# jetuk/pycllp

Hardware: AMD Instinct MI355X
Metric: LPs solved/sec (higher is better)
Workload: dtype f64

## Files before the change

pycllp_amd/csrc/ipm_group.inc:

```

#ifndef PYCLLP_SPLITJ
#define PYCLLP_SPLITJ 6
#endif
#ifndef PYCLLP_GRAM_UNROLL
#define PYCLLP_GRAM_UNROLL 4
#endif
#ifndef PYCLLP_AT_RB
#define PYCLLP_AT_RB 4
#endif
#ifndef PYCLLP_A_CB
#define PYCLLP_A_CB 8
#endif
#ifndef PYCLLP_SOLVE_PRIO
#define PYCLLP_SOLVE_PRIO 2
#endif
#ifndef PYCLLP_FACTOR_PRIO
#define PYCLLP_FACTOR_PRIO 2
#endif
#ifndef PYCLLP_FACTOR_PRIO_HSD
#define PYCLLP_FACTOR_PRIO_HSD 3
#endif
#ifndef PYCLLP_WPB
#define PYCLLP_WPB 8
#endif
// ... 51 lines not shown
    static constexpr int GTAB_OFF = AIMG + ND;
    __device__ static void fill_gram_table(double* lds, int tid, int nthreads) {
        if constexpr (MP == 32) {
            unsigned short* tab = (unsigned short*)(lds + GTAB_OFF);
            for (int i = tid; i < GROWS * 64; i += nthreads)
                tab[i] = (unsigned short)(i < GRAM_INSTS * 64 ? gram_store(i >> 6, i & 63) : gram_wrap(i & 63));
        }
    }
    static constexpr int SHARED = GTAB_OFF + GTAB;
    static constexpr int WSZ = G * SLAB + STAGE_SZ;
    static constexpr size_t lds_bytes(int wpb) { return sizeof(double) * (size_t)(SHARED + wpb * WSZ); }
    __host__ __device__ static constexpr int kpos(int j) { return (j & 3) * KS + (j >> 2); }
};

template <int MP>
__device__ __forceinline__ double grp_sum(double v) {
    asm volatile("" : "+v"(v));
    v += dpp_d<0xB1>(v);
    v += dpp_d<0x4E>(v);
    v += dpp_d<0x141>(v);
    v += dpp_d<0x140>(v);
    if (MP == 32) v = row_pair_sum(v);
    return v;
}
template <int MP>
__device__ __forceinline__ double grp_max(double v) {
    v = fmax(v, dpp_d<0xB1>(v));
    v = fmax(v, dpp_d<0x4E>(v));
    v = fmax(v, dpp_d<0x141>(v));
    v = fmax(v, dpp_d<0x140>(v));
    if (MP == 32) v = row_pair_max(v);
    return v;
}
template <int MP>
__device__ __forceinline__ double grp_bcast(double v, int k, int grp) {
    if (MP == 32) {
        const double a = readlane_d(v, k), b = readlane_d(v, 32 + k);
        return grp ? b : a;
    } else {
        const double a = readlane_d(v, k), b = readlane_d(v, 16 + k), c = readlane_d(v, 32 + k), d = readlane_d(v, 48 + k);
        return (grp & 2) ? ((grp & 1) ? d : c) : ((grp & 1) ? b : a);
    }
}

template <int MP, int NP, bool SL = false>
struct GWave {
    using G_ = GeoG<MP, NP, SL>;
    static constexpr int G = G_::G, NCG = G_::NCG, NCD = G_::NCD, ND = G_::ND, JB = G_::JB, KS = G_::KS, AS = G_::AS, MS = G_::MS;

    const double* Aimg;
    static constexpr bool COLB = MP == 32 && NP <= 96;
    static constexpr bool ROWB = COLB && SL;
    static constexpr bool CARRY = COLB || MP == 16;
    unsigned rb[ROWB ? 16 : 1];
    unsigned xb[COLB ? 16 : 1];
    double* slab;
    double* slab0;
    double* stage;
    int lane, gl, grp, m, n;

    __device__ __forceinline__ int ogl() const { int g = gl; asm volatile("" : "+v"(g)); return g; }

    __device__ __forceinline__ void load_own_row(double (&out)[MP]) const {
        typedef double double2_t __attribute__((ext_vector_type(2)));
        if constexpr (ROWB) {
#pragma unroll
            for (int p2 = 0; p2 < MP / 2; p2++) {
                const double2_t t = *(const __attribute__((address_space(3))) double2_t*)(size_t)rb[p2];
                out[2 * p2] = t[0]; out[2 * p2 + 1] = t[1];
            }
            return;
        }
        const int g = ogl();
        const double2_t* rp = (const double2_t*)(slab + g * MS);
        const int g15 = G_::SWZ ? (g & 15) : 0;
#pragma unroll
        for (int p2 = 0; p2 < MP / 2; p2++) {
            const double2_t t = rp[p2 ^ g15];
            out[2 * p2] = t[0]; out[2 * p2 + 1] = t[1];
        }
    }

    template <bool STAGED = false>
    __device__ __forceinline__ void At_times(double u, double (&out)[NCG]) const {
        const int g = ogl();
        double ur[2] = {u, u};
        const __attribute__((address_space(3))) double* ub = nullptr;
        if constexpr (STAGED) {
            stage[grp * MP + g] = u;
            wave_lds_sync();
            unsigned uba = lds_addr(stage + grp * MP);
            asm volatile("" : "+v"(uba));
            ub = (const __attribute__((address_space(3))) double*)(size_t)uba;
        } else if constexpr (MP == 32) {
            ur[0] = top_row_d(u); ur[1] = bottom_row_d(u);
        }
        const double* ac = Aimg + g;
        constexpr int RB = PYCLLP_AT_RB, NB = MP / RB;
        double a0[RB][NCD], a1[RB][NCD], u0[RB], u1[RB];
#define AT_LOAD(A_, U_, I0)                                                                     \
    static_for<0, RB>([&](auto ic_) {                                                           \
        constexpr int ii = decltype(ic_)::value, i_ = (I0) + ii;                                \
        if constexpr (STAGED) U_[ii] = ub[i_ + tok];                                            \
        else U_[ii] = row_bcast<(i_ & 15)>(ur[i_ >> 4]);                                        \
        _Pragma("unroll") for (int q = 0; q < NCD; q++) A_[ii][q] = ac[i_ * AS + MP * q + tok]; \
    });
#define AT_USE(A_, U_)                                                                          \
    _Pragma("unroll") for (int ii = 0; ii < RB; ii++) {                                         \
        asm volatile("" : "+v"(U_[ii]));                                                        \
        _Pragma("unroll") for (int q = 0; q < NCD; q++) asm volatile("" : "+v"(A_[ii][q]));     \
    }                                                                                           \
    asm volatile("" : "+v"(tok));                                                               \
    _Pragma("unroll") for (int ii = 0; ii < RB; ii++)                                           \
        _Pragma("unroll") for (int q = 0; q < NCD; q++) out[q] = fma(A_[ii][q], U_[ii], out[q]); \
    _Pragma("unroll") for (int q = 0; q < NCD; q++) asm volatile("" : "+v"(out[q]));
#pragma unroll
        for (int q = 0; q < NCG; q++) out[q] = 0.0;
        if (SL) out[NCG - 1] = u;
        int tok = 0;
        asm volatile("" : "+v"(tok));
        AT_LOAD(a0, u0, 0)
        static_for<0, NB / 2>([&](auto bc) {
            constexpr int b2 = 2 * decltype(bc)::value;
            AT_LOAD(a1, u1, (b2 + 1) * RB)
            AT_USE(a0, u0)
            if constexpr (b2 + 2 < NB) { AT_LOAD(a0, u0, (b2 + 2) * RB) }
            AT_USE(a1, u1)
        });
#undef AT_LOAD
#undef AT_USE
        if constexpr (STAGED) wave_lds_sync();
    }
// ... 79 lines not shown
                    acc[0] = __builtin_amdgcn_mfma_f64_4x4x4f64(ad[0], a[0], acc[0], 0, 0, 0);
                    acc[1] = __builtin_amdgcn_mfma_f64_4x4x4f64(ad[1], a[1], acc[1], 0, 0, 0);
                    acc[2] = __builtin_amdgcn_mfma_f64_4x4x4f64(ad[0], p3, acc[2], 0, 0, 0);
                    acc[3] = __builtin_amdgcn_mfma_f64_4x4x4f64(ad[1], p7, acc[3], 0, 0, 0);
                    acc[4] = __builtin_amdgcn_mfma_f64_4x4x4f64(top ? ad[0] : ad[1], p2, acc[4], 0, 0, 0);
                }
            }
            int lo_ = lane;
            asm volatile("" : "+v"(lo_));
            if constexpr (LATE) {
                const unsigned short* tab2 = (const unsigned short*)(Aimg + G_::GTAB_OFF) + lo_;
#pragma unroll
                for (int r = 0; r < GRAM_INSTS; r++) so[r] = tab2[64 * r];
            }
            const unsigned sga = lds_addr(sg);
#pragma unroll
            for (int r = 0; r < GRAM_INSTS; r++) *(__attribute__((address_space(3))) double*)(size_t)(sga + so[r]) = acc[r];
            const int kg2 = lo_ >> 4, c0 = (lo_ & 15) ^ (kg2 << 1);
            double* e0 = sg + kg2 * G_::MS + c0;
            double* e1 = sg + kg2 * G_::MS + (c0 ^ 8);
#pragma unroll
            for (int r4 = 0; r4 < 4; r4++) ((r4 & 1) ? e1 : e0)[(16 + 4 * r4) * G_::MS + 16 * (r4 >> 1)] = acc10[r4];
        } else {
            double4_t acc = (double4_t){0.0, 0.0, 0.0, 0.0};
#pragma unroll PYCLLP_GRAM_UNROLL
            for (int s0 = 0; s0 < KS; s0 += SC) {
#pragma unroll
                for (int ss = 0; ss < SC; ss++) {
                    const int s = s0 + ss;
                    const double xk = AX ? px[s] : 0.0, dk = pd[s], tk = pt[s];
                    const double a = arow[4 * s];
                    if (AX) axp[0] = fma(a, xk, axp[0]);
                    adp[0] = fma(a, tk, adp[0]);
                    acc = __builtin_amdgcn_mfma_f64_16x16x4f64(a * dk, a, acc, 0, 0, 0);
                }
            }
            int lo_ = lane;
            asm volatile("" : "+v"(lo_));
            const int kg2 = lo_ >> 4, cc2 = lo_ & 15;
#pragma unroll
            for (int r4 = 0; r4 < 4; r4++) sg[G_::sidx(kg2 + 4 * r4, cc2)] = acc[r4];
        }
        if constexpr (MP == 32) {
            if (AX) ax = quad_sum2(axp[0], axp[1]);
            ad = quad_sum2(adp[0], adp[1]);
        } else {
            if (AX) ax = quad_sum(axp[0]);
            ad = quad_sum(adp[0]);
        }
    }

    __device__ __forceinline__ static double top_row_of(double u) { return top_row_d(u); }

    template <bool RELF = false>
    __device__ __forceinline__ bool factor_dpp(double (&W)[MP], double beta2, double floor_, bool live, double& rdiag,
                                               const double* fl = nullptr) const {
        return factor_sweep<RELF, 0>(W, beta2, floor_, live, rdiag, fl, nullptr);
    }
    template <bool RELF = false, int NR>
    __device__ __forceinline__ bool factor_dpp_fwd(double (&W)[MP], double beta2, double floor_, bool live, double& rdiag,
                                                   double (&r)[NR], const double* fl = nullptr) const {
        return factor_sweep<RELF, NR>(W, beta2, floor_, live, rdiag, fl, r);
    }
    template <int OP, int NR>
    __device__ __forceinline__ static void fwd_bottom_op(const double (&W)[MP], double* r, const double* so, double* a) {
        if constexpr (OP >= 0 && OP < 16) {
#pragma unroll
            for (int i = 0; i < NR; i++) dot_step<OP, 0xA>(a[i], so[i], W[OP]);
        } else if constexpr (OP == 16) {
#pragma unroll
            for (int i = 0; i < NR; i++) r[i] -= a[i];
        } else if constexpr (OP > 16 && OP < 32) {
#pragma unroll
            for (int i = 0; i < NR; i++) fwd_step<OP - 17, 0xA>(r[i], W[OP - 1]);
        }
    }
    template <bool RELF, int NR>
    __device__ __forceinline__ bool factor_sweep(double (&W)[MP], double beta2, double floor_, bool live, double& rdiag,
                                                 const double* fl, double* r) const {
        rdiag = 1.0;
        constexpr int PRIO_ = RELF ? PYCLLP_FACTOR_PRIO_HSD : PYCLLP_FACTOR_PRIO;
        if constexpr (PRIO_ != 0) __builtin_amdgcn_s_setprio(PRIO_);
        const int go = ogl();
        (void)go;
        constexpr int NR1 = NR ? NR : 1;
        double so[NR1], acc[NR1];
#pragma unroll
        for (int i = 0; i < NR1; i++) { so[i] = 0.0; acc[i] = 0.0; }
        double ymax = 0.0;
        static_for<0, MP>([&](auto jc) {
            constexpr int j = decltype(jc)::value;
            const double u = W[j];
            double src = u;
            if constexpr (MP == 32 && j < 16) src = top_row_of(u);
            const double piv = bcast64<j % 16>(src);
            if constexpr (NR > 0 && MP == 32 && j > 16) fwd_bottom_op<2 * (j - 16) - 1, NR>(W, r, so, acc);
            const double aD = RELF ? max_abs<false>(piv, fl[j]) : max_abs<true>(piv, floor_);
            double rD = fast_rcp(aD);
            if constexpr (NR > 0 && MP == 32 && j >= 16) {
                asm volatile("" : "+v"(rD));
                fwd_bottom_op<2 * (j - 16), NR>(W, r, so, acc);
            }
            constexpr unsigned below32 = (j + 1 < 32) ? (0xFFFFFFFFu << ((j + 1) & 31)) : 0u;
            constexpr unsigned below16 = (j + 1 < 16) ? (((0xFFFFu << ((j + 1) & 15)) & 0xFFFFu) * 0x10001u) : 0u;
            constexpr unsigned MB_ = (MP == 32) ? below32 : below16;
            constexpr unsigned ONE_ = (MP == 32) ? (1u << (j % 32)) : ((1u << (j % 16)) * 0x10001u);
            double l = 0.0;
            asm volatile("" : "+v"(l));
            if constexpr (MP == 16) {
                chain_step_exec<j, MB_, MB_, 1, ONE_, ONE_>(W, 0.0, rD, l, ymax, rdiag);
            } else if constexpr (j < 16) {
                chain_step_exec<j, MB_, MB_, 0, ONE_, ONE_>(*reinterpret_cast<double (*)[16]>(&W[0]), src, rD, l, ymax, rdiag);
                chain_all_neg(*reinterpret_cast<double (*)[16]>(&W[16]), W[j], l);
            } else {
                chain_step_exec<j - 16, MB_, MB_, 1, ONE_, ONE_>(*reinterpret_cast<double (*)[16]>(&W[16]), 0.0, rD, l, ymax, rdiag);
            }
            W[j] = l;
            if constexpr (COLB) *(__attribute__((address_space(3))) double*)(size_t)(xb[j & 15] + 256u * (unsigned)(j & ~15)) = l;
            else if constexpr (MP == 16) slab[G_::sidx(j, go)] = l;
            if constexpr (NR > 0 && j < 15) {
#pragma unroll
                for (int i = 0; i < NR; i++) fwd_step<j, (MP == 32) ? 0x5 : 0xF>(r[i], l);
                if constexpr (MP == 32 && j == 14) {
#pragma unroll
                    for (int i = 0; i < NR; i++) so[i] = top_row_d(r[i]);
                }
            }
        });
        if constexpr (NR > 0 && MP == 32) fwd_bottom_op<31, NR>(W, r, so, acc);
        const bool viol = live && (ymax > beta2);
        if constexpr (PRIO_ != 0) __builtin_amdgcn_s_setprio(0);
        if constexpr (!CARRY) {
            const int g = ogl();
#pragma unroll
            for (int j = 0; j < MP; j++) slab[G_::sidx(j, g)] = W[j];
        }
        wave_lds_sync();
        return __any(viol);
    }

    __device__ __forceinline__ double factor_guarded_inplace(bool rowok, double beta2, double floor_,
                                                             const double* fl = nullptr) const {
        if (!rowok) slab[G_::sidx(gl, gl)] = 1.0;
        wave_lds_sync();
        double rdiag = 1.0;
#pragma unroll 1
        for (int j = 0; j < MP; j++) {
            const bool below = gl > j;
            const double u = below ? slab[G_::sidx(gl, j)] : 0.0;
            const double piv = slab[G_::sidx(j, j)];
            const double theta = grp_max<MP>(fabs(u));
            const double aD = fmax(fmax(fabs(piv), fl ? fl[j] : floor_), theta * theta / beta2);
            const double rD = fast_rcp(aD);
            const double li = u * rD;
            if (gl == j) rdiag = rD;
#pragma unroll 1
            for (int k = j + 1; k < MP; k++) {
                const double uk = slab[G_::sidx(k, j)];
                if (gl >= k) slab[G_::sidx(gl, k)] = fma(-li, uk, slab[G_::sidx(gl, k)]);
            }
            wave_lds_sync();
            slab[G_::sidx(j, gl)] = below ? li : 0.0;
            wave_lds_sync();
        }
#pragma unroll 1
        for (int k = 0; k < MP; k++) if (k <= gl) slab[G_::sidx(gl, k)] = 0.0;
        wave_lds_sync();
        return rdiag;
    }

    __device__ __forceinline__ double fwd_back(double s, double rdiag) const {
        if constexpr (PYCLLP_SOLVE_PRIO != 0) __builtin_amdgcn_s_setprio(PYCLLP_SOLVE_PRIO);
        forward(s);
        backward(s, rdiag);
        if constexpr (MP == 32 && PYCLLP_SOLVE_PRIO != 0) __builtin_amdgcn_s_setprio(0);
        return s;
    }
    __device__ __forceinline__ double back_after_sweep(double s, double rdiag) const {
        if constexpr (PYCLLP_SOLVE_PRIO != 0) __builtin_amdgcn_s_setprio(PYCLLP_SOLVE_PRIO);
        backward(s, rdiag);
// ... 253 lines not shown
                    if (fin_e) finalize(stat_e);
                    continue;
                }
            }
        }
        STAMP(0)

        double Ax = 0.0, Adt = 0.0;
        double rxk[NCG], rzk[NCG];
#pragma unroll
        for (int q = 0; q < NCG; q++) { rxk[q] = fast_rcp(x[q]); rzk[q] = fast_rcp(z[q]); }
        auto do_gram = [&](double& Ax_, double& Adt_) {
            double d[NCG], t[NCG];
#pragma unroll
            for (int q = 0; q < NCG; q++) {
                const double rx = rxk[q], rz = rzk[q];
                d[q] = ok[q] ? x[q] * rz : 0.0;
                t[q] = ok[q] ? c[q] - v[q] + mu * rx : 0.0;
            }
#pragma unroll 1
            for (int g = 0; g < G; g++) {
                if (__shfl((int)live, g * MP, WAVE) == 0) continue;
                const bool carried = __shfl((int)have_pred, g * MP, WAVE) != 0;
                if (grp == g) {
#pragma unroll
                    for (int q = 0; q < NCD; q++) {
                        const int p = G_::kpos(gl + MP * q);
                        if (!carried) w.stage[p] = ok[q] ? x[q] : 0.0;
                        w.stage[ND + p] = d[q];
                        w.stage[2 * ND + p] = d[q] * t[q];
                    }
                }
                wave_lds_sync();
                double axg = 0.0, adg;
                if (carried) w.template gram_one<false>(g, axg, adg); else w.template gram_one<true>(g, axg, adg);
                wave_lds_sync();
                if (grp == g) { Ax_ = axg; Adt_ = adg; }
            }
            if (SL) {
                Ax_ += ok[NCG - 1] ? x[NCG - 1] : 0.0;
                Adt_ += d[NCG - 1] * t[NCG - 1];
                w.slab[G_::sidx(gl, gl)] += d[NCG - 1];
                wave_lds_sync();
            }
        };
        do_gram(Ax, Adt);
        STAMP(2)
        const double rho = have_pred ? rho_pred : b - Ax;
        const double rhs = Adt - rho;
        double rdiag;
        double fs[1] = {rhs};
        constexpr bool CARRY = GWave<MP, NP, SL>::CARRY && !(PC && SL && MP == 32 && NP == 96);
        bool fused = CARRY;
        {
            double W[MP];
            const int gd = w.ogl();
            if (m < MP) {
                if (!rowok) w.slab[G_::sidx(gd, gd)] = 1.0;
                wave_lds_sync();
            }
            w.load_own_row(W);
            double diag = rowok ? w.slab[G_::sidx(gd, gd)] : 0.0;
            const double beta2 = grp_max<MP>(fabs(diag));
            wave_lds_sync();
            STAMP(3)
            bool redo;
            if constexpr (CARRY) redo = w.factor_dpp_fwd(W, beta2, o.pivot_floor, live, rdiag, fs);
            else redo = w.factor_dpp(W, beta2, o.pivot_floor, live, rdiag);
            if (redo || (o.flags & PYCLLP_FLAG_FORCE_GUARD_PATH)) {
                double Ax2, Adt2;
                do_gram(Ax2, Adt2);
                rdiag = w.factor_guarded_inplace(rowok, beta2, o.pivot_floor);
                fused = false;
            }
            STAMP(4)
        }
        double cor[NCG];
        double rhs_c = rhs;
        if constexpr (PC) {
            const double dya = fused ? w.back_after_sweep(fs[0], rdiag) : w.fwd_back(rhs, rdiag);
            double wva[NCG], dxa[NCG], dza[NCG], dt[NCG];
            w.At_times(dya, wva);
            double tha = 0.0;
#pragma unroll
            for (int q = 0; q < NCG; q++) {
                const double rx = rxk[q], rz = rzk[q];
                const double dq = ok[q] ? x[q] * rz : 0.0;
                const double ta = ok[q] ? c[q] - v[q] : 0.0;
                dxa[q] = (ta - wva[q]) * dq;
                dza[q] = ok[q] ? (-z[q] * dxa[q]) * rx - z[q] : 0.0;
                if (ok[q]) tha = fmax(tha, fmax(-dza[q] * rz, -dxa[q] * rx));
            }
            tha = grp_max<MP>(tha);
            const double theta_a = fmin(1.0 / tha, 1.0);
            double ga = 0.0;
#pragma unroll
            for (int q = 0; q < NCG; q++) ga += ok[q] ? fma(theta_a, dxa[q], x[q]) * fma(theta_a, dza[q], z[q]) : 0.0;
            ga = grp_sum<MP>(ga);
            const double sg = ga / gam;
            mu = sg * sg * sg * gam / (double)n;
#pragma unroll
            for (int q = 0; q < NCG; q++) {
                const double rx = rxk[q], rz = rzk[q];
                cor[q] = ok[q] ? mu - dxa[q] * dza[q] : 0.0;
                const double tq = ok[q] ? c[q] - v[q] + cor[q] * rx : 0.0;
                dt[q] = (ok[q] ? x[q] * rz : 0.0) * tq;
            }
            rhs_c = w.A_times(dt) - rho;
        }
        double dy = (!PC && fused) ? w.back_after_sweep(fs[0], rdiag) : w.fwd_back(rhs_c, rdiag);
        STAMP(5)
        double wv[NCG], dx[NCG], d[NCG];
        w.At_times(dy, wv);
#pragma unroll
        for (int q = 0; q < NCG; q++) {
            const double rx = rxk[q], rz = rzk[q];
            d[q] = ok[q] ? x[q] * rz : 0.0;
            const double tq = ok[q] ? c[q] - v[q] + (PC ? cor[q] : mu) * rx : 0.0;
            dx[q] = (tq - wv[q]) * d[q];
        }
        STAMP(6)
// ... 65 lines not shown
```

pycllp_amd/csrc/ipm_group_hsd.inc:

```

#ifndef PYCLLP_HSD_AT_RB
#define PYCLLP_HSD_AT_RB 4
#endif
template <int MP, int NP, bool SL>
struct GWaveH : GWave<MP, NP, SL> {
    using Base = GWave<MP, NP, SL>;
    using G_ = GeoG<MP, NP, SL>;
    static constexpr int G = G_::G, NCG = G_::NCG, NCD = G_::NCD, AS = G_::AS, MS = G_::MS;

    template <bool STAGED = false>
    __device__ __forceinline__ void At_times2(double u1, double u2, double (&o1)[NCG], double (&o2)[NCG]) const {
        const int g = this->ogl();
        double ur1[2] = {u1, u1}, ur2[2] = {u2, u2};
        const __attribute__((address_space(3))) double* ub = nullptr;
        if constexpr (STAGED) {
            this->stage[this->grp * MP + g] = u1;
            this->stage[G * MP + this->grp * MP + g] = u2;
            wave_lds_sync();
            unsigned uba = lds_addr(this->stage + this->grp * MP);
            asm volatile("" : "+v"(uba));
            ub = (const __attribute__((address_space(3))) double*)(size_t)uba;
        } else if constexpr (MP == 32) {
            ur1[0] = top_row_d(u1); ur1[1] = bottom_row_d(u1);
            ur2[0] = top_row_d(u2); ur2[1] = bottom_row_d(u2);
// ... 305 lines not shown
            if (__any(fin_e)) {
                if (fin_e) finalize(stat_e);
                continue;
            }
        }

        const double mu = (gam + tau * kap) / (double)(iopaque(n) + 1), dmu = o.delta * mu;
        const double phi = du - po + kap;
        po_prev = po; du_prev = du;

        double Adc = 0.0, Adr = 0.0;
        auto do_gram = [&](double& Adc_, double& Adr_) {
            double d[NCG], r1[NCG];
#pragma unroll
            for (int q = 0; q < NCG; q++) {
                const double rx = fast_rcp(x[q]), rz = fast_rcp(z[q]);
                const double sg = fma(c[q], tau, z[q] - v[q]);
                d[q] = ok[q] ? x[q] * rz : 0.0;
                r1[q] = ok[q] ? fma(HSD_ETA, sg, fma(dmu, rx, -z[q])) : 0.0;
            }
            const int go = w.ogl();
#pragma unroll 1
            for (int g = 0; g < G; g++) {
                if (__shfl((int)live, g * MP, WAVE) == 0) continue;
                if (grp == g) {
#pragma unroll
                    for (int q = 0; q < NCD; q++) {
                        const int p = G_::kpos(go + MP * q);
                        w.stage[p] = d[q] * c[q];
                        w.stage[ND + p] = d[q];
                        w.stage[2 * ND + p] = d[q] * r1[q];
                    }
                }
                wave_lds_sync();
                double axg, adg;
                w.gram_one(g, axg, adg);
                wave_lds_sync();
                if (grp == g) { Adc_ = axg; Adr_ = adg; }
            }
            if (SL) {
                Adc_ += d[NCG - 1] * c[NCG - 1];
                Adr_ += d[NCG - 1] * r1[NCG - 1];
                w.slab[G_::sidx(go, go)] += d[NCG - 1];
                wave_lds_sync();
            }
        };
        do_gram(Adc, Adr);
        double pv = Adc - b;
        double qv = fma(-HSD_ETA, rho, Adr);
        double rdiag;
        constexpr bool CARRY = GWave<MP, NP, SL>::CARRY;
        double fr[2] = {pv, qv};
        bool fused = CARRY;
        {
            double W[MP];
            const int go = w.ogl();
            if (m < MP) {
                if (!rowok) w.slab[G_::sidx(go, go)] = 1.0;
                wave_lds_sync();
            }
            w.load_own_row(W);
            double diag = rowok ? w.slab[G_::sidx(go, go)] : 0.0;
            const double beta2 = grp_max<MP>(fabs(diag));
            int gro = grp;
            asm volatile("" : "+v"(gro));
            double* fl = w.stage + gro * MP;
            const double pf = sopaque(o.pivot_floor);
            const double myfloor = pf * pf * fabs(diag);
            fl[go] = myfloor;
            wave_lds_sync();
            bool redo;
            if constexpr (CARRY) redo = w.template factor_dpp_fwd<true>(W, beta2, 0.0, live, rdiag, fr, fl);
            else redo = w.template factor_dpp<true>(W, beta2, 0.0, live, rdiag, fl);
            if (redo || (o.flags & PYCLLP_FLAG_FORCE_GUARD_PATH)) {
                double t1, t2;
                do_gram(t1, t2);
                fl[go] = myfloor;
                wave_lds_sync();
                rdiag = w.factor_guarded_inplace(rowok, beta2, 0.0, fl);
                fused = false;
            }
        }
        if (fused) { pv = fr[0]; qv = fr[1]; w.backward2(pv, qv, rdiag); }
        else w.fwd_back2(pv, qv, rdiag);
        double ap[NCG], aq[NCG], dx[NCG], d[NCG], wv[NCG];
        constexpr bool AT_STAGED = MP == 32 && NP == 128 && !SL;
        w.template At_times2<AT_STAGED>(pv, qv, ap, aq);
        double dsum = 0.0, nsum = 0.0;
#pragma unroll
        for (int q = 0; q < NCG; q++) {
            const double rx = fast_rcp(x[q]), rz = fast_rcp(z[q]);
            const double sg = fma(c[q], tau, z[q] - v[q]);
            d[q] = ok[q] ? x[q] * rz : 0.0;
            const double r1 = ok[q] ? fma(HSD_ETA, sg, fma(dmu, rx, -z[q])) : 0.0;
            const double cp = c[q] - ap[q];
            const double u = d[q] * cp;
            dx[q] = d[q] * (r1 - aq[q]);
            ap[q] = u;
            wv[q] = cp;
            dsum = fma(u, cp, dsum);
            nsum = fma(c[q], dx[q], nsum);
        }
        const double den = grp_sum<MP>(dsum) + kap / tau;
        const double num = fma(HSD_ETA, phi, dmu / tau - kap) + grp_sum<MP>(b * qv) - grp_sum<MP>(nsum);
        const double dtau = num / den;
        double dy = fma(pv, dtau, qv);
#pragma unroll
        for (int q = 0; q < NCG; q++) {
            dx[q] = fma(ap[q], dtau, dx[q]);
            wv[q] = fma(c[q] - wv[q], dtau, aq[q]);
        }
        const double etol = o.refine_tol * (1.0 + nb) * fmax(tau, kap);
        const double rhs_e = fma(b, dtau, HSD_ETA * rho);
        int nref = 0;
        double e;
        for (;;) {
            e = rhs_e - w.A_times(dx);
            const double maxe = grp_max<MP>(fabs(e));
            const bool need = live && (maxe > etol) && (nref < o.max_refine);
            if (!__any(need)) break;
            const double ec = w.fwd_back(need ? e : 0.0, rdiag);
            double w2[NCG];
            w.At_times(ec, w2);
#pragma unroll
            for (int q = 0; q < NCG; q++) {
                dx[q] = fma(d[q], w2[q], dx[q]);
// ... 40 lines not shown
```

pycllp_amd/csrc/ipm_group_slot_body.inc:

```
    using G_ = GeoG<MP, NP, SL>;
    using P_ = GeoPA<G_>;
    constexpr int G = G_::G, NCG = G_::NCG, NCD = G_::NCD, ND = G_::ND, JB = G_::JB, AS = G_::AS;
    static_assert(SL || !BD, "the bounded equality form ends in the identity");
    const int nd = SL ? n - m : n;
    extern __shared__ __attribute__((aligned(16))) double lds[];
    const int tid = threadIdx.x;
    const int wpb = blockDim.x / WAVE;
    if constexpr (!PA) {
        for (int i = tid; i < G_::AIMG; i += blockDim.x) {
            const int r = i / AS, cidx = i % AS;
            lds[i] = (r < m && cidx < nd) ? Ag[(size_t)r * n + cidx] : 0.0;
        }
        G_::fill_gram_table(lds, tid, blockDim.x);
        __syncthreads();
        for (int j = tid; j < ND; j += blockDim.x) {
            double sacc = 0.0;
            for (int i = 0; i < MP; i++) sacc += lds[i * AS + j];
            lds[G_::AIMG + j] = sacc;
        }
        __syncthreads();
    }

    GWave<MP, NP, SL> w;
    const int wave = tid / WAVE;
// ... 254 lines not shown
            dq = a ? dq : 0.0;
            tq = a ? tq : 0.0;
        };
        auto do_gram = [&](double& Ax_, double& Adt_) {
            double d[NCG], tt[NCG];
#pragma unroll
            for (int q = 0; q < NCG; q++) newton_dt(q, d[q], tt[q]);
#pragma unroll 1
            for (int g = 0; g < G; g++) {
                if (__shfl((int)live, g * MP, WAVE) == 0) continue;
                if (grp == g) {
#pragma unroll
                    for (int q = 0; q < NCD; q++) {
                        const int p = G_::kpos(gl + MP * q);
                        w.stage[p] = act(q) ? x[q] : 0.0;
                        w.stage[ND + p] = d[q];
                        w.stage[2 * ND + p] = d[q] * tt[q];
                    }
                }
                wave_lds_sync();
                double axg, adg;
                if constexpr (PA) w.Aimg = areas + g * P_::AREA;
                w.template gram_one<true, true>(g, axg, adg);
                if constexpr (PA) w.Aimg = own_area;
                wave_lds_sync();
                if (grp == g) { Ax_ = axg; Adt_ = adg; }
            }
            if (SL) {
                Ax_ += act(NCG - 1) ? x[NCG - 1] : 0.0;
                Adt_ += d[NCG - 1] * tt[NCG - 1];
                w.slab[G_::sidx(gl, gl)] += d[NCG - 1];
                wave_lds_sync();
            }
        };
        double Ax = 0.0, Adt = 0.0;
        do_gram(Ax, Adt);
        const double rho = b - Ax;
        const double normr = sqrt(grp_sum<MP>(rho * rho));

        int stat = PYCLLP_STATUS_ITERATION_LIMIT;
        bool fin = true;
        if (!(isfinite(normr) && isfinite(norms) && isfinite(gam) && (!BD || isfinite(ntau)))) stat = PYCLLP_STATUS_NUMERICAL;
        else if (normr <= tol_r && norms <= tol_s && gam <= o.eps * (1.0 + fabs(po)) && (!BD || ntau <= tol_u)) stat = PYCLLP_STATUS_OPTIMAL;
        else if (normr > 10.0 * normr0 && normr > PYCLLP_GROWTH_FLOOR * tol_r) stat = PYCLLP_STATUS_PRIMAL_INFEASIBLE;
        else if (norms > 10.0 * norms0 && norms > PYCLLP_GROWTH_FLOOR * tol_s) stat = PYCLLP_STATUS_DUAL_INFEASIBLE;
        else fin = false;
        const bool work = live && !fin;

        const double rhs = Adt - rho;
        double rdiag;
        constexpr bool CARRY = GWave<MP, NP, SL>::CARRY;
        double fs[1] = {rhs};
        bool fused = CARRY;
        {
            double W[MP];
            const int gd = w.ogl();
            if (m < MP) {
                if (!rowok) w.slab[G_::sidx(gd, gd)] = 1.0;
                wave_lds_sync();
            }
            w.load_own_row(W);
            double diag = rowok ? w.slab[G_::sidx(gd, gd)] : 0.0;
            const double beta2 = grp_max<MP>(fabs(diag));
            wave_lds_sync();
            bool redo;
            if constexpr (CARRY) redo = w.factor_dpp_fwd(W, beta2, o.pivot_floor, work, rdiag, fs);
            else redo = w.factor_dpp(W, beta2, o.pivot_floor, work, rdiag);
            if (redo || (o.flags & PYCLLP_FLAG_FORCE_GUARD_PATH)) {
                double Ax2, Adt2;
                do_gram(Ax2, Adt2);
                rdiag = w.factor_guarded_inplace(rowok, beta2, o.pivot_floor);
                fused = false;
            }
        }
        double dy = fused ? w.back_after_sweep(fs[0], rdiag) : w.fwd_back(rhs, rdiag);
        double wv[NCG], dx[NCG], d[NCG];
        w.At_times(dy, wv);
#pragma unroll
        for (int q = 0; q < NCG; q++) {
            double tq;
            newton_dt(q, d[q], tq);
            dx[q] = (tq - wv[q]) * d[q];
        }
        int nref = 0;
        for (;;) {
            const double e = rho - w.A_times(dx);
            const double maxe = grp_max<MP>(fabs(e));
            const bool need = work && (maxe > etol) && (nref < o.max_refine);
            if (!__any(need)) break;
            const double eta = w.fwd_back(need ? e : 0.0, rdiag);
            double w2[NCG];
            w.At_times(eta, w2);
#pragma unroll
            for (int q = 0; q < NCG; q++) {
                dx[q] = fma(d[q], w2[q], dx[q]);
                wv[q] -= w2[q];
            }
            dy -= eta;
            nref += need ? 1 : 0;
        }
        const unsigned long long nf = __ballot(!isfinite(dy));
        const bool dy_bad = ((nf >> (grp * MP)) & gmask) != 0ull;
        if (!fin && dy_bad) { fin = true; stat = PYCLLP_STATUS_NUMERICAL; }

        if (!fin) {
            double dz[NCG], dt[NCG], ds[NCG];
            double th = 0.0;
#pragma unroll
            for (int q = 0; q < NCG; q++) {
                const bool a = act(q), bq = bnd(q);
                const double tau = BD ? (u[q] - x[q]) - t[q] : 0.0;
                dz[q] = a ? (mu - z[q] * dx[q]) * rxk[q] - z[q] : 0.0;
                dt[q] = bq ? tau - dx[q] : 0.0;
                ds[q] = bq ? (mu - s[q] * dt[q]) * rtk[q] - s[q] : 0.0;
                if (act(q)) th = fmax(th, fmax(-dz[q] * rzk[q], -dx[q] * rxk[q]));
                if (bq) th = fmax(th, fmax(-dt[q] * rtk[q], -ds[q] * fast_rcp(s[q])));
            }
            th = grp_max<MP>(th);
            const double theta = fmin(o.r / th, 1.0);
            y = fma(theta, dy, y);
// ... 18 lines not shown
```

pycllp_amd/csrc/wave_common.h:

```cpp
#ifndef PYCLLP_WAVE_COMMON_H
#define PYCLLP_WAVE_COMMON_H
#include <hip/hip_runtime.h>
#include <math.h>
#include <stdio.h>
#include <string.h>

#include <algorithm>
#include <atomic>
#include <mutex>
#include <unordered_map>
#include <type_traits>
#include <vector>

#include "../../include/pycllp_hip.h"

#define PYCLLP_GROWTH_FLOOR 1e3

typedef double double4_t __attribute__((ext_vector_type(4)));

inline hipError_t set_dyn_lds(const void* fn, int bytes) {
    static std::mutex mu;
    static std::unordered_map<unsigned long long, int> done;
    int dev = 0;
    (void)hipGetDevice(&dev);
// ... 123 lines not shown
                 CHAIN_COL_FMA(0, J_) \
                 CHAIN_COL_FMA(1, J_) \
                 CHAIN_COL_FMA(2, J_) \
                 CHAIN_COL_FMA(3, J_) \
                 CHAIN_COL_FMA(4, J_) \
                 CHAIN_COL_FMA(5, J_) \
                 CHAIN_COL_FMA(6, J_) \
                 CHAIN_COL_FMA(7, J_) \
                 CHAIN_COL_FMA(8, J_) \
                 CHAIN_COL_FMA(9, J_) \
                 CHAIN_COL_FMA(10, J_) \
                 CHAIN_COL_FMA(11, J_) \
                 CHAIN_COL_FMA(12, J_) \
                 CHAIN_COL_FMA(13, J_) \
                 CHAIN_COL_FMA(14, J_) \
                 CHAIN_COL_FMA(15, J_) \
                 "s_mov_b64 exec, %19" \
                 : "+v"(Wd[0]), "+v"(Wd[1]), "+v"(Wd[2]), "+v"(Wd[3]), "+v"(Wd[4]), "+v"(Wd[5]), "+v"(Wd[6]), "+v"(Wd[7]), "+v"(Wd[8]), "+v"(Wd[9]), "+v"(Wd[10]), "+v"(Wd[11]), "+v"(Wd[12]), "+v"(Wd[13]), "+v"(Wd[14]), "+v"(Wd[15]), \
                   "+v"(l), "+v"(ymax), "=&v"(t), "=&s"(save), "+v"(rdiag) \
                 : "v"(src), "v"(rD), "n"(MLO), "n"(MHI), "n"(SELF), "n"(ONELO), "n"(ONEHI)); \
}
DEF_CHAIN_COL(0) DEF_CHAIN_COL(1) DEF_CHAIN_COL(2) DEF_CHAIN_COL(3) DEF_CHAIN_COL(4) DEF_CHAIN_COL(5) DEF_CHAIN_COL(6) DEF_CHAIN_COL(7)
DEF_CHAIN_COL(8) DEF_CHAIN_COL(9) DEF_CHAIN_COL(10) DEF_CHAIN_COL(11) DEF_CHAIN_COL(12) DEF_CHAIN_COL(13) DEF_CHAIN_COL(14) DEF_CHAIN_COL(15)
#undef DEF_CHAIN_COL
#undef CHAIN_COL_FMA
template <int J, unsigned MLO, unsigned MHI, int SELF, unsigned ONELO, unsigned ONEHI>
__device__ __forceinline__ void chain_step_exec(double (&Wd)[16], double src, double rD, double& l, double& ymax, double& rdiag) {
#define CHAIN_COL_CASE(J_) if constexpr (J == J_) chain_col_##J_<MLO, MHI, SELF, ONELO, ONEHI>(Wd, src, rD, l, ymax, rdiag);
    CHAIN_COL_CASE(0) CHAIN_COL_CASE(1) CHAIN_COL_CASE(2) CHAIN_COL_CASE(3) CHAIN_COL_CASE(4) CHAIN_COL_CASE(5) CHAIN_COL_CASE(6) CHAIN_COL_CASE(7)
    CHAIN_COL_CASE(8) CHAIN_COL_CASE(9) CHAIN_COL_CASE(10) CHAIN_COL_CASE(11) CHAIN_COL_CASE(12) CHAIN_COL_CASE(13) CHAIN_COL_CASE(14) CHAIN_COL_CASE(15)
#undef CHAIN_COL_CASE
}
__device__ __forceinline__ void chain_all_neg(double (&Wd)[16], double src, double l) {
    asm volatile("s_nop 1\n\t"
                 "v_fmac_f64_dpp %0, %16, -%17 row_newbcast:0 row_mask:0xf bank_mask:0xf\n\t"
                 "v_fmac_f64_dpp %1, %16, -%17 row_newbcast:1 row_mask:0xf bank_mask:0xf\n\t"
                 "v_fmac_f64_dpp %2, %16, -%17 row_newbcast:2 row_mask:0xf bank_mask:0xf\n\t"
                 "v_fmac_f64_dpp %3, %16, -%17 row_newbcast:3 row_mask:0xf bank_mask:0xf\n\t"
                 "v_fmac_f64_dpp %4, %16, -%17 row_newbcast:4 row_mask:0xf bank_mask:0xf\n\t"
                 "v_fmac_f64_dpp %5, %16, -%17 row_newbcast:5 row_mask:0xf bank_mask:0xf\n\t"
                 "v_fmac_f64_dpp %6, %16, -%17 row_newbcast:6 row_mask:0xf bank_mask:0xf\n\t"
                 "v_fmac_f64_dpp %7, %16, -%17 row_newbcast:7 row_mask:0xf bank_mask:0xf\n\t"
                 "v_fmac_f64_dpp %8, %16, -%17 row_newbcast:8 row_mask:0xf bank_mask:0xf\n\t"
                 "v_fmac_f64_dpp %9, %16, -%17 row_newbcast:9 row_mask:0xf bank_mask:0xf\n\t"
                 "v_fmac_f64_dpp %10, %16, -%17 row_newbcast:10 row_mask:0xf bank_mask:0xf\n\t"
                 "v_fmac_f64_dpp %11, %16, -%17 row_newbcast:11 row_mask:0xf bank_mask:0xf\n\t"
                 "v_fmac_f64_dpp %12, %16, -%17 row_newbcast:12 row_mask:0xf bank_mask:0xf\n\t"
                 "v_fmac_f64_dpp %13, %16, -%17 row_newbcast:13 row_mask:0xf bank_mask:0xf\n\t"
                 "v_fmac_f64_dpp %14, %16, -%17 row_newbcast:14 row_mask:0xf bank_mask:0xf\n\t"
                 "v_fmac_f64_dpp %15, %16, -%17 row_newbcast:15 row_mask:0xf bank_mask:0xf\n\t"
                 : "+v"(Wd[0]), "+v"(Wd[1]), "+v"(Wd[2]), "+v"(Wd[3]), "+v"(Wd[4]), "+v"(Wd[5]), "+v"(Wd[6]), "+v"(Wd[7]), "+v"(Wd[8]), "+v"(Wd[9]), "+v"(Wd[10]), "+v"(Wd[11]), "+v"(Wd[12]), "+v"(Wd[13]), "+v"(Wd[14]), "+v"(Wd[15])
                 : "v"(src), "v"(l));
}
template <bool BS>
__device__ __forceinline__ double max_abs(double a, double b) {
    double r;
    if constexpr (BS) asm volatile("v_max_f64 %0, |%1|, %2" : "=v"(r) : "v"(a), "s"(b));
    else asm volatile("v_max_f64 %0, |%1|, %2" : "=v"(r) : "v"(a), "v"(b));
    return r;
}
template <unsigned M16, unsigned ONE16>
__device__ __forceinline__ void chain_head_exec(double u, double rD, double& nli, double& ymax, double& rdiag) {
    double t;
    unsigned long long save;
    asm volatile("v_mov_b64 %0, 0\n\t"
                 "s_mov_b64 %4, exec\n\ts_mov_b32 exec_lo, %7\n\ts_mov_b32 exec_hi, %7\n\t"
                 "v_mul_f64 %0, -%5, %6\n\t"
                 "v_mul_f64 %3, %0, %5\n\t"
                 "v_max_f64 %1, %1, |%3|\n\t"
                 "s_mov_b32 exec_lo, %8\n\ts_mov_b32 exec_hi, %8\n\t"
                 "v_mov_b64 %2, %6\n\t"
                 "s_mov_b64 exec, %4"
                 : "=&v"(nli), "+v"(ymax), "+v"(rdiag), "=&v"(t), "=&s"(save)
                 : "v"(u), "v"(rD), "n"(M16), "n"(ONE16));
}
template <unsigned MLO, unsigned MHI>
__device__ __forceinline__ void mov_exec(double& dst, double v) {
    unsigned long long save;
    asm volatile("s_mov_b64 %1, exec\n\ts_mov_b32 exec_lo, %3\n\ts_mov_b32 exec_hi, %4\n\tv_mov_b64 %0, %2\n\ts_mov_b64 exec, %1"
                 : "+v"(dst), "=&s"(save) : "v"(v), "n"(MLO), "n"(MHI));
}

__device__ __forceinline__ void subst15_up(double& s, const double* l) {
    asm volatile("s_nop 1\n\tv_fmac_f64_dpp %0, %0, -%1 row_newbcast:0 row_mask:0xf bank_mask:0xf\n\t"
                 "s_nop 1\n\tv_fmac_f64_dpp %0, %0, -%2 row_newbcast:1 row_mask:0xf bank_mask:0xf\n\t"
                 "s_nop 1\n\tv_fmac_f64_dpp %0, %0, -%3 row_newbcast:2 row_mask:0xf bank_mask:0xf\n\t"
                 "s_nop 1\n\tv_fmac_f64_dpp %0, %0, -%4 row_newbcast:3 row_mask:0xf bank_mask:0xf\n\t"
                 "s_nop 1\n\tv_fmac_f64_dpp %0, %0, -%5 row_newbcast:4 row_mask:0xf bank_mask:0xf\n\t"
                 "s_nop 1\n\tv_fmac_f64_dpp %0, %0, -%6 row_newbcast:5 row_mask:0xf bank_mask:0xf\n\t"
                 "s_nop 1\n\tv_fmac_f64_dpp %0, %0, -%7 row_newbcast:6 row_mask:0xf bank_mask:0xf\n\t"
                 "s_nop 1\n\tv_fmac_f64_dpp %0, %0, -%8 row_newbcast:7 row_mask:0xf bank_mask:0xf\n\t"
                 "s_nop 1\n\tv_fmac_f64_dpp %0, %0, -%9 row_newbcast:8 row_mask:0xf bank_mask:0xf\n\t"
                 "s_nop 1\n\tv_fmac_f64_dpp %0, %0, -%10 row_newbcast:9 row_mask:0xf bank_mask:0xf\n\t"
                 "s_nop 1\n\tv_fmac_f64_dpp %0, %0, -%11 row_newbcast:10 row_mask:0xf bank_mask:0xf\n\t"
                 "s_nop 1\n\tv_fmac_f64_dpp %0, %0, -%12 row_newbcast:11 row_mask:0xf bank_mask:0xf\n\t"
                 "s_nop 1\n\tv_fmac_f64_dpp %0, %0, -%13 row_newbcast:12 row_mask:0xf bank_mask:0xf\n\t"
                 "s_nop 1\n\tv_fmac_f64_dpp %0, %0, -%14 row_newbcast:13 row_mask:0xf bank_mask:0xf\n\t"
                 "s_nop 1\n\tv_fmac_f64_dpp %0, %0, -%15 row_newbcast:14 row_mask:0xf bank_mask:0xf\n\t"
                 : "+v"(s) : "v"(l[0]), "v"(l[1]), "v"(l[2]), "v"(l[3]), "v"(l[4]), "v"(l[5]), "v"(l[6]), "v"(l[7]), "v"(l[8]), "v"(l[9]), "v"(l[10]), "v"(l[11]), "v"(l[12]), "v"(l[13]), "v"(l[14]));
}
__device__ __forceinline__ void subst15_down(double& s, const double* l) {
    asm volatile("s_nop 1\n\tv_fmac_f64_dpp %0, %0, -%1 row_newbcast:15 row_mask:0xf bank_mask:0xf\n\t"
                 "s_nop 1\n\tv_fmac_f64_dpp %0, %0, -%2 row_newbcast:14 row_mask:0xf bank_mask:0xf\n\t"
                 "s_nop 1\n\tv_fmac_f64_dpp %0, %0, -%3 row_newbcast:13 row_mask:0xf bank_mask:0xf\n\t"
                 "s_nop 1\n\tv_fmac_f64_dpp %0, %0, -%4 row_newbcast:12 row_mask:0xf bank_mask:0xf\n\t"
                 "s_nop 1\n\tv_fmac_f64_dpp %0, %0, -%5 row_newbcast:11 row_mask:0xf bank_mask:0xf\n\t"
// ... 96 lines not shown
                 "v_fmac_f64_dpp %0, %1, %15 row_newbcast:13 row_mask:0xf bank_mask:0xf\n\t"
                 "v_fmac_f64_dpp %0, %1, %16 row_newbcast:14 row_mask:0xf bank_mask:0xf\n\t"
                 "v_fmac_f64_dpp %0, %1, %17 row_newbcast:15 row_mask:0xf bank_mask:0xf\n\t"
                 : "+v"(a) : "v"(src), "v"(l[0]), "v"(l[1]), "v"(l[2]), "v"(l[3]), "v"(l[4]), "v"(l[5]), "v"(l[6]), "v"(l[7]), "v"(l[8]), "v"(l[9]), "v"(l[10]), "v"(l[11]), "v"(l[12]), "v"(l[13]), "v"(l[14]), "v"(l[15]));
    return a;
}

template <int K, int RM>
__device__ __forceinline__ void fwd_step(double& s, double l) {
    asm volatile("s_nop 1\n\tv_fmac_f64_dpp %0, %0, -%1 row_newbcast:" DPP_STR(%2) " row_mask:" DPP_STR(%3) " bank_mask:0xf"
                 : "+v"(s) : "v"(l), "n"(K), "n"(RM));
}
template <int K, int RM>
__device__ __forceinline__ void dot_step(double& a, double src, double l) {
    if constexpr (K == 0)
        asm volatile("s_nop 1\n\tv_fmac_f64_dpp %0, %1, %2 row_newbcast:" DPP_STR(%3) " row_mask:" DPP_STR(%4) " bank_mask:0xf"
                     : "+v"(a) : "v"(src), "v"(l), "n"(K), "n"(RM));
    else
        asm volatile("v_fmac_f64_dpp %0, %1, %2 row_newbcast:" DPP_STR(%3) " row_mask:" DPP_STR(%4) " bank_mask:0xf"
                     : "+v"(a) : "v"(src), "v"(l), "n"(K), "n"(RM));
}

__device__ __forceinline__ double quad_sum(double v) {
    int lo = __double2loint(v), hi = __double2hiint(v);
    auto a = __builtin_amdgcn_permlane16_swap(lo, lo, false, false);
    auto b = __builtin_amdgcn_permlane16_swap(hi, hi, false, false);
    v = __hiloint2double(b[0], a[0]) + __hiloint2double(b[1], a[1]);
    lo = __double2loint(v); hi = __double2hiint(v);
    auto c = __builtin_amdgcn_permlane32_swap(lo, lo, false, false);
    auto d = __builtin_amdgcn_permlane32_swap(hi, hi, false, false);
    return __hiloint2double(d[0], c[0]) + __hiloint2double(d[1], c[1]);
}
__device__ __forceinline__ double quad_sum2(double a, double b) {
    auto l = __builtin_amdgcn_permlane16_swap(__double2loint(a), __double2loint(b), false, false);
    auto h = __builtin_amdgcn_permlane16_swap(__double2hiint(a), __double2hiint(b), false, false);
    const double v = __hiloint2double(h[0], l[0]) + __hiloint2double(h[1], l[1]);
    const int lo = __double2loint(v), hi = __double2hiint(v);
    auto c = __builtin_amdgcn_permlane32_swap(lo, lo, false, false);
    auto d = __builtin_amdgcn_permlane32_swap(hi, hi, false, false);
    return __hiloint2double(d[0], c[0]) + __hiloint2double(d[1], c[1]);
}
__device__ __forceinline__ double top_row_d(double v) {
    const int lo = __double2loint(v), hi = __double2hiint(v);
    auto a = __builtin_amdgcn_permlane16_swap(lo, lo, false, false);
    auto b = __builtin_amdgcn_permlane16_swap(hi, hi, false, false);
    return __hiloint2double(b[0], a[0]);
}
__device__ __forceinline__ double bottom_row_d(double v) {
    const int lo = __double2loint(v), hi = __double2hiint(v);
    auto a = __builtin_amdgcn_permlane16_swap(lo, lo, false, false);
    auto b = __builtin_amdgcn_permlane16_swap(hi, hi, false, false);
    return __hiloint2double(b[1], a[1]);
}
__device__ __forceinline__ double row_pair_sum(double v) {
    const int lo = __double2loint(v), hi = __double2hiint(v);
    auto a = __builtin_amdgcn_permlane16_swap(lo, lo, false, false);
    auto b = __builtin_amdgcn_permlane16_swap(hi, hi, false, false);
    return __hiloint2double(b[0], a[0]) + __hiloint2double(b[1], a[1]);
}
__device__ __forceinline__ double row_pair_max(double v) {
    const int lo = __double2loint(v), hi = __double2hiint(v);
    auto a = __builtin_amdgcn_permlane16_swap(lo, lo, false, false);
    auto b = __builtin_amdgcn_permlane16_swap(hi, hi, false, false);
    return fmax(__hiloint2double(b[0], a[0]), __hiloint2double(b[1], a[1]));
}
__device__ __forceinline__ double row_sum(double v) {
    asm volatile("" : "+v"(v));
    v += dpp_d<0xB1>(v);
    v += dpp_d<0x4E>(v);
    v += dpp_d<0x141>(v);
    v += dpp_d<0x140>(v);
    return v;
}
__device__ __forceinline__ void row_sum4(double (&v)[4]) {
#define ROW_SUM4_STAGE(C)                                                                      \
    {                                                                                          \
        double t_[4];                                                                          \
        _Pragma("unroll") for (int i = 0; i < 4; i++) t_[i] = dpp_d<C>(v[i]);                  \
        _Pragma("unroll") for (int i = 0; i < 4; i++) asm volatile("" : "+v"(t_[i]));          \
        _Pragma("unroll") for (int i = 0; i < 4; i++) v[i] += t_[i];                           \
        _Pragma("unroll") for (int i = 0; i < 4; i++) asm volatile("" : "+v"(v[i]));           \
    }
#pragma unroll
    for (int i = 0; i < 4; i++) asm volatile("" : "+v"(v[i]));
    ROW_SUM4_STAGE(0xB1) ROW_SUM4_STAGE(0x4E) ROW_SUM4_STAGE(0x141) ROW_SUM4_STAGE(0x140)
#undef ROW_SUM4_STAGE
}
__device__ __forceinline__ double row_max(double v) {
    v = fmax(v, dpp_d<0xB1>(v));
    v = fmax(v, dpp_d<0x4E>(v));
    v = fmax(v, dpp_d<0x141>(v));
    v = fmax(v, dpp_d<0x140>(v));
    return v;
}
__device__ __forceinline__ double uni(double v) {
    return __hiloint2double(__builtin_amdgcn_readfirstlane(__double2hiint(v)), __builtin_amdgcn_readfirstlane(__double2loint(v)));
}
__device__ __forceinline__ double wsum(double v) {
    v = row_sum(v);
    return uni((readlane_d(v, 0) + readlane_d(v, 16)) + (readlane_d(v, 32) + readlane_d(v, 48)));
}
__device__ __forceinline__ double wmax(double v) {
    v = row_max(v);
    return uni(fmax(fmax(readlane_d(v, 0), readlane_d(v, 16)), fmax(readlane_d(v, 32), readlane_d(v, 48))));
}

// ... 72 lines not shown
```

Measured before the change: 12.41 million.

## Split MP=32 Cholesky sweep across lane halves with LDS merge

For 32-row groups, the factor sweep's first 16 pivots now update only half of the trailing block (W[24..31]) per lane, using a rearranged row load that gives top lanes data from a different part of the slab. After pivot 15, the halves are merged through LDS so the second phase sees a consistent W[16..23]. This cuts the number of DPP fused multiply-adds in the first phase by roughly half. In exchange it adds permlane/DPP shuffles, an extra LDS store/sync/load round, and intricate address arithmetic that could be wrong.

```diff
diff --git a/pycllp_amd/csrc/ipm_group.inc b/pycllp_amd/csrc/ipm_group.inc
--- a/pycllp_amd/csrc/ipm_group.inc
+++ b/pycllp_amd/csrc/ipm_group.inc
@@ -127,6 +127,7 @@
     static constexpr bool COLB = MP == 32 && NP <= 96;
     static constexpr bool ROWB = COLB && SL;
     static constexpr bool CARRY = COLB || MP == 16;
+    static constexpr bool SPLIT = MP == 32;
     unsigned rb[ROWB ? 16 : 1];
     unsigned xb[COLB ? 16 : 1];
     double* slab;
@@ -153,6 +154,75 @@
         for (int p2 = 0; p2 < MP / 2; p2++) {
             const double2_t t = rp[p2 ^ g15];
             out[2 * p2] = t[0]; out[2 * p2 + 1] = t[1];
+        }
+    }
+
+    __device__ __forceinline__ static unsigned top_lanes(int g) { return (((unsigned)g >> 4) & 1u) - 1u; }
+    __device__ __forceinline__ static unsigned split_off(int g) {
+        return (5952u - (((unsigned)g & 8u) << 9) + (((unsigned)g & 12u) << 5)) & top_lanes(g);
+    }
+    __device__ __forceinline__ static unsigned split_row(int g) { return ((24u - 2u * ((unsigned)g & 8u)) * (unsigned)(MS / 2)) & top_lanes(g); }
+    __device__ __forceinline__ static int split_swz(int g) { return (g & 15) ^ (int)(12u & top_lanes(g)); }
+    template <bool SP = SPLIT>
+    __device__ __forceinline__ void load_row_for_sweep(double (&out)[MP]) const {
+        if constexpr (!SP) {
+            load_own_row(out);
+        } else {
+            typedef double double2_t __attribute__((ext_vector_type(2)));
+            const int g = ogl();
+            if constexpr (ROWB) {
+                const unsigned off = split_off(g);
+#pragma unroll
+                for (int p2 = 0; p2 < MP / 2; p2++) {
+                    const double2_t t = *(const __attribute__((address_space(3))) double2_t*)(size_t)(rb[p2] + (p2 >= 12 ? off : 0u));
+                    out[2 * p2] = t[0]; out[2 * p2 + 1] = t[1];
+                }
+            } else {
+                const double2_t* rp = (const double2_t*)(slab + g * MS);
+                const int g15 = g & 15;
+                const double2_t* rs = rp + split_row(g);
+                const int g15s = split_swz(g);
+#pragma unroll
+                for (int p2 = 0; p2 < MP / 2; p2++) {
+                    const double2_t t = p2 >= 12 ? rs[p2 ^ g15s] : rp[p2 ^ g15];
+                    out[2 * p2] = t[0]; out[2 * p2 + 1] = t[1];
+                }
+            }
+        }
+    }
+
+    __device__ __forceinline__ void merge_through_slab(double (&W)[MP]) const {
+        typedef double double2_t __attribute__((ext_vector_type(2)));
+        const int g = ogl();
+        if constexpr (ROWB) {
+            const unsigned off = split_off(g);
+#pragma unroll
+            for (int q = 0; q < 4; q++) {
+                double2_t t; t[0] = W[24 + 2 * q]; t[1] = W[25 + 2 * q];
+                *(__attribute__((address_space(3))) double2_t*)(size_t)(rb[12 + q] + off) = t;
+            }
+            wave_lds_sync();
+#pragma unroll
+            for (int q = 0; q < 4; q++) {
+                const double2_t t = *(const __attribute__((address_space(3))) double2_t*)(size_t)rb[8 + q];
+                W[16 + 2 * q] = t[0]; W[17 + 2 * q] = t[1];
+            }
+        } else {
+            double2_t* rp = (double2_t*)(slab + g * MS);
+            const int g15 = g & 15;
+            double2_t* rs = rp + split_row(g);
+            const int g15s = split_swz(g);
+#pragma unroll
+            for (int q = 0; q < 4; q++) {
+                double2_t t; t[0] = W[24 + 2 * q]; t[1] = W[25 + 2 * q];
+                rs[(12 + q) ^ g15s] = t;
+            }
+            wave_lds_sync();
+#pragma unroll
+            for (int q = 0; q < 4; q++) {
+                const double2_t t = rp[(8 + q) ^ g15];
+                W[16 + 2 * q] = t[0]; W[17 + 2 * q] = t[1];
+            }
         }
     }
 
@@ -338,15 +408,15 @@
 
     __device__ __forceinline__ static double top_row_of(double u) { return top_row_d(u); }
 
-    template <bool RELF = false>
+    template <bool RELF = false, bool SP = SPLIT>
     __device__ __forceinline__ bool factor_dpp(double (&W)[MP], double beta2, double floor_, bool live, double& rdiag,
                                                const double* fl = nullptr) const {
-        return factor_sweep<RELF, 0>(W, beta2, floor_, live, rdiag, fl, nullptr);
-    }
-    template <bool RELF = false, int NR>
+        return factor_sweep<RELF, 0, SP>(W, beta2, floor_, live, rdiag, fl, nullptr);
+    }
+    template <bool RELF = false, bool SP = SPLIT, int NR>
     __device__ __forceinline__ bool factor_dpp_fwd(double (&W)[MP], double beta2, double floor_, bool live, double& rdiag,
                                                    double (&r)[NR], const double* fl = nullptr) const {
-        return factor_sweep<RELF, NR>(W, beta2, floor_, live, rdiag, fl, r);
+        return factor_sweep<RELF, NR, SP>(W, beta2, floor_, live, rdiag, fl, r);
     }
     template <int OP, int NR>
     __device__ __forceinline__ static void fwd_bottom_op(const double (&W)[MP], double* r, const double* so, double* a) {
@@ -361,7 +431,7 @@
             for (int i = 0; i < NR; i++) fwd_step<OP - 17, 0xA>(r[i], W[OP - 1]);
         }
     }
-    template <bool RELF, int NR>
+    template <bool RELF, int NR, bool SP>
     __device__ __forceinline__ bool factor_sweep(double (&W)[MP], double beta2, double floor_, bool live, double& rdiag,
                                                  const double* fl, double* r) const {
         rdiag = 1.0;
@@ -378,7 +448,9 @@
             constexpr int j = decltype(jc)::value;
             const double u = W[j];
             double src = u;
-            if constexpr (MP == 32 && j < 16) src = top_row_of(u);
+            double ub = u;
+            if constexpr (SP && j < 16) src = both_rows_d(u, ub);
+            else if constexpr (MP == 32 && j < 16) src = top_row_of(u);
             const double piv = bcast64<j % 16>(src);
             if constexpr (NR > 0 && MP == 32 && j > 16) fwd_bottom_op<2 * (j - 16) - 1, NR>(W, r, so, acc);
             const double aD = RELF ? max_abs<false>(piv, fl[j]) : max_abs<true>(piv, floor_);
@@ -397,7 +469,8 @@
                 chain_step_exec<j, MB_, MB_, 1, ONE_, ONE_>(W, 0.0, rD, l, ymax, rdiag);
             } else if constexpr (j < 16) {
                 chain_step_exec<j, MB_, MB_, 0, ONE_, ONE_>(*reinterpret_cast<double (*)[16]>(&W[0]), src, rD, l, ymax, rdiag);
-                chain_all_neg(*reinterpret_cast<double (*)[16]>(&W[16]), W[j], l);
+                if constexpr (SP) chain_half_neg(*reinterpret_cast<double (*)[8]>(&W[24]), ror8_top_d(ub), rD);
+                else chain_all_neg(*reinterpret_cast<double (*)[16]>(&W[16]), W[j], l);
             } else {
                 chain_step_exec<j - 16, MB_, MB_, 1, ONE_, ONE_>(*reinterpret_cast<double (*)[16]>(&W[16]), 0.0, rD, l, ymax, rdiag);
             }
@@ -412,6 +485,7 @@
                     for (int i = 0; i < NR; i++) so[i] = top_row_d(r[i]);
                 }
             }
+            if constexpr (SP && j == 15) merge_through_slab(W);
         });
         if constexpr (NR > 0 && MP == 32) fwd_bottom_op<31, NR>(W, r, so, acc);
         const bool viol = live && (ymax > beta2);
@@ -771,6 +845,7 @@
         double fs[1] = {rhs};
         constexpr bool CARRY = GWave<MP, NP, SL>::CARRY && !(PC && SL && MP == 32 && NP == 96);
         bool fused = CARRY;
+        constexpr bool SPLIT = GWave<MP, NP, SL>::SPLIT && !(PC && SL && MP == 32 && NP == 96);
         {
             double W[MP];
             const int gd = w.ogl();
@@ -778,14 +853,14 @@
                 if (!rowok) w.slab[G_::sidx(gd, gd)] = 1.0;
                 wave_lds_sync();
             }
-            w.load_own_row(W);
+            w.template load_row_for_sweep<SPLIT>(W);
             double diag = rowok ? w.slab[G_::sidx(gd, gd)] : 0.0;
             const double beta2 = grp_max<MP>(fabs(diag));
             wave_lds_sync();
             STAMP(3)
             bool redo;
-            if constexpr (CARRY) redo = w.factor_dpp_fwd(W, beta2, o.pivot_floor, live, rdiag, fs);
-            else redo = w.factor_dpp(W, beta2, o.pivot_floor, live, rdiag);
+            if constexpr (CARRY) redo = w.template factor_dpp_fwd<false, SPLIT>(W, beta2, o.pivot_floor, live, rdiag, fs);
+            else redo = w.template factor_dpp<false, SPLIT>(W, beta2, o.pivot_floor, live, rdiag);
             if (redo || (o.flags & PYCLLP_FLAG_FORCE_GUARD_PATH)) {
                 double Ax2, Adt2;
                 do_gram(Ax2, Adt2);
diff --git a/pycllp_amd/csrc/ipm_group_hsd.inc b/pycllp_amd/csrc/ipm_group_hsd.inc
--- a/pycllp_amd/csrc/ipm_group_hsd.inc
+++ b/pycllp_amd/csrc/ipm_group_hsd.inc
@@ -381,6 +381,7 @@
         constexpr bool CARRY = GWave<MP, NP, SL>::CARRY;
         double fr[2] = {pv, qv};
         bool fused = CARRY;
+        constexpr bool SPLIT = GWave<MP, NP, SL>::SPLIT;
         {
             double W[MP];
             const int go = w.ogl();
@@ -388,7 +389,7 @@
                 if (!rowok) w.slab[G_::sidx(go, go)] = 1.0;
                 wave_lds_sync();
             }
-            w.load_own_row(W);
+            w.template load_row_for_sweep<SPLIT>(W);
             double diag = rowok ? w.slab[G_::sidx(go, go)] : 0.0;
             const double beta2 = grp_max<MP>(fabs(diag));
             int gro = grp;
@@ -399,8 +400,8 @@
             fl[go] = myfloor;
             wave_lds_sync();
             bool redo;
-            if constexpr (CARRY) redo = w.template factor_dpp_fwd<true>(W, beta2, 0.0, live, rdiag, fr, fl);
-            else redo = w.template factor_dpp<true>(W, beta2, 0.0, live, rdiag, fl);
+            if constexpr (CARRY) redo = w.template factor_dpp_fwd<true, SPLIT>(W, beta2, 0.0, live, rdiag, fr, fl);
+            else redo = w.template factor_dpp<true, SPLIT>(W, beta2, 0.0, live, rdiag, fl);
             if (redo || (o.flags & PYCLLP_FLAG_FORCE_GUARD_PATH)) {
                 double t1, t2;
                 do_gram(t1, t2);
diff --git a/pycllp_amd/csrc/ipm_group_slot_body.inc b/pycllp_amd/csrc/ipm_group_slot_body.inc
--- a/pycllp_amd/csrc/ipm_group_slot_body.inc
+++ b/pycllp_amd/csrc/ipm_group_slot_body.inc
@@ -330,6 +330,7 @@
         constexpr bool CARRY = GWave<MP, NP, SL>::CARRY;
         double fs[1] = {rhs};
         bool fused = CARRY;
+        constexpr bool SPLIT = GWave<MP, NP, SL>::SPLIT && !(BD && PA && MP == 32 && NP == 96);
         {
             double W[MP];
             const int gd = w.ogl();
@@ -337,13 +338,13 @@
                 if (!rowok) w.slab[G_::sidx(gd, gd)] = 1.0;
                 wave_lds_sync();
             }
-            w.load_own_row(W);
+            w.template load_row_for_sweep<SPLIT>(W);
             double diag = rowok ? w.slab[G_::sidx(gd, gd)] : 0.0;
             const double beta2 = grp_max<MP>(fabs(diag));
             wave_lds_sync();
             bool redo;
-            if constexpr (CARRY) redo = w.factor_dpp_fwd(W, beta2, o.pivot_floor, work, rdiag, fs);
-            else redo = w.factor_dpp(W, beta2, o.pivot_floor, work, rdiag);
+            if constexpr (CARRY) redo = w.template factor_dpp_fwd<false, SPLIT>(W, beta2, o.pivot_floor, work, rdiag, fs);
+            else redo = w.template factor_dpp<false, SPLIT>(W, beta2, o.pivot_floor, work, rdiag);
             if (redo || (o.flags & PYCLLP_FLAG_FORCE_GUARD_PATH)) {
                 double Ax2, Adt2;
                 do_gram(Ax2, Adt2);
diff --git a/pycllp_amd/csrc/wave_common.h b/pycllp_amd/csrc/wave_common.h
--- a/pycllp_amd/csrc/wave_common.h
+++ b/pycllp_amd/csrc/wave_common.h
@@ -199,6 +199,21 @@
                  : "+v"(Wd[0]), "+v"(Wd[1]), "+v"(Wd[2]), "+v"(Wd[3]), "+v"(Wd[4]), "+v"(Wd[5]), "+v"(Wd[6]), "+v"(Wd[7]), "+v"(Wd[8]), "+v"(Wd[9]), "+v"(Wd[10]), "+v"(Wd[11]), "+v"(Wd[12]), "+v"(Wd[13]), "+v"(Wd[14]), "+v"(Wd[15])
                  : "v"(src), "v"(l));
 }
+__device__ __forceinline__ void chain_half_neg(double (&Wd)[8], double x, double rD) {
+    double lx;
+    asm volatile("v_mul_f64 %8, %9, %10\n\t"
+                 "s_nop 0\n\t"
+                 "v_fmac_f64_dpp %0, %9, -%8 row_newbcast:8 row_mask:0xf bank_mask:0xf\n\t"
+                 "v_fmac_f64_dpp %1, %9, -%8 row_newbcast:9 row_mask:0xf bank_mask:0xf\n\t"
+                 "v_fmac_f64_dpp %2, %9, -%8 row_newbcast:10 row_mask:0xf bank_mask:0xf\n\t"
+                 "v_fmac_f64_dpp %3, %9, -%8 row_newbcast:11 row_mask:0xf bank_mask:0xf\n\t"
+                 "v_fmac_f64_dpp %4, %9, -%8 row_newbcast:12 row_mask:0xf bank_mask:0xf\n\t"
+                 "v_fmac_f64_dpp %5, %9, -%8 row_newbcast:13 row_mask:0xf bank_mask:0xf\n\t"
+                 "v_fmac_f64_dpp %6, %9, -%8 row_newbcast:14 row_mask:0xf bank_mask:0xf\n\t"
+                 "v_fmac_f64_dpp %7, %9, -%8 row_newbcast:15 row_mask:0xf bank_mask:0xf\n\t"
+                 : "+v"(Wd[0]), "+v"(Wd[1]), "+v"(Wd[2]), "+v"(Wd[3]), "+v"(Wd[4]), "+v"(Wd[5]), "+v"(Wd[6]), "+v"(Wd[7]), "=&v"(lx)
+                 : "v"(x), "v"(rD));
+}
 template <bool BS>
 __device__ __forceinline__ double max_abs(double a, double b) {
     double r;
@@ -401,6 +416,19 @@
     auto b = __builtin_amdgcn_permlane16_swap(hi, hi, false, false);
     return __hiloint2double(b[1], a[1]);
 }
+__device__ __forceinline__ double both_rows_d(double v, double& bot) {
+    const int lo = __double2loint(v), hi = __double2hiint(v);
+    auto a = __builtin_amdgcn_permlane16_swap(lo, lo, false, false);
+    auto b = __builtin_amdgcn_permlane16_swap(hi, hi, false, false);
+    bot = __hiloint2double(b[1], a[1]);
+    return __hiloint2double(b[0], a[0]);
+}
+__device__ __forceinline__ double ror8_top_d(double v) {
+    int lo = __double2loint(v), hi = __double2hiint(v);
+    lo = __builtin_amdgcn_update_dpp(lo, lo, 0x128, 0x5, 0xF, false);
+    hi = __builtin_amdgcn_update_dpp(hi, hi, 0x128, 0x5, 0xF, false);
+    return __hiloint2double(hi, lo);
+}
 __device__ __forceinline__ double row_pair_sum(double v) {
     const int lo = __double2loint(v), hi = __double2hiint(v);
     auto a = __builtin_amdgcn_permlane16_swap(lo, lo, false, false);
```

Measured after the change: 12.63 million, median of 6. 1.7% higher.
